# jmschrei/PyPore

Hardware: AMD Instinct MI355X
Metric: Msamples/sec segmented (SpeedyStatSplit, 10^8-sample trace); %HBM roofline (higher is better)
Workload: dtype int32/f64 (exact integer block sums of fp32 or int16 samples; decisions in fp64)

## Files before the change

pypore_amd/csrc/poreseg.hip:

```cpp
#include <hip/hip_runtime.h>

#include <algorithm>
#include <chrono>
#include <complex>
#include <cmath>
#include <cstdarg>
#include <cstdio>
#include <cstdlib>
#include <cstring>
#include <condition_variable>
#include <mutex>
#include <string>
#include <thread>
#include <tuple>
#include <vector>

#include "poreseg.h"
#include "seg_device.hpp"
#include "seg_align.hpp"
#include "seg_pairwise.hpp"
#include "seg_hmm.hpp"

using namespace ps;

// ... 62 lines not shown
    int tree_mw = 0;
    int upload_by_kernel = 1;
    int filter_fused = 1;
    int k0_waves = 0;
    float noise_k = 0.1f;
    int k0_admit = 0;
    int k0_sets = 2;
    bool chain_held = false;
    unsigned long long chain_ticket = 0;
    bool defer_sync = false;
    int scan_lds_pad = 0;
    int k0_unaligned = 1;
    int single_pass = 1;
    int gather_fused = 1;
    int download_by_kernel = 1;
    int debug = 0;
#ifdef PS_DIAG
    int dbg_phase = 0;
    int dbg_k0_nogrp = 0;
#endif
    int k0_shared = 0;
    hipEvent_t ev_front[2] = {};
    bool stream_idle = true;
    int tree_par = 1;
    int groups = 1;
    int scan_bs = 1;
    int wide_bs = 1;
    int bridge_single = 1 << 30;
    int tree_tail_pct = 0;
    int slots_pct = 100;
// ... 29 lines not shown
    DevBuf bridges, bmeta, tile_i32, sp_off, spine_items, asm_hdr, ev_first_tile;
    DevBuf bridge_ext, ext_slot, ext_list;
    DevBuf lat_state, lat_seam, lat_res;
    unsigned lat_tag_next = 1;
    unsigned lat_tag_base = 0;
    int lat_help = 1;
    int bridge_budget = BR_MAX;
    int bridge_ext_on = 1;
    HostBuf h_hdr;
    DevBuf spine_jobs, spine_scratch, spine_dense, spine_meta, tree_jobs, tree_scratch, tree_spill,
        tree_counts, items, item_pos, first_item, ev_off, bounds_off, small;
    HostBuf h_meta, h_dense, h_small, h_up;
    hipEvent_t ev[10] = {};
    int timing = 1;
    double ms[8] = {0, 0, 0, 0, 0, 0, 0, 0};
    int64_t counters[14] = {0, 0, 0, 0, 0, 0, 0, 0, 0, 0, 0, 0, 0, 0};
};

namespace {

int fail(ps_ctx *ctx, int code, const char *fmt, ...)
{
    if (ctx) {
        char buf[512];
        va_list ap;
        va_start(ap, fmt);
        vsnprintf(buf, sizeof buf, fmt, ap);
        va_end(ap);
        ctx->err = buf;
    }
    return code;
// ... 51 lines not shown
        if (c.gen[w % K0Chain::RING] == w + 1) HIP_TRY(ctx, hipStreamWaitEvent(st, c.ev[w % K0Chain::RING], 0));
    }
    return PS_OK;
}
int chain_publish(ps_ctx *ctx, int device, hipStream_t st, unsigned long long ticket)
{
    K0Chain &c = g_chain[device & 15];
    std::lock_guard<std::mutex> lk(c.mu);
    HIP_TRY(ctx, hipEventRecord(c.ev[ticket % K0Chain::RING], st));
    c.gen[ticket % K0Chain::RING] = ticket + 1;
    return PS_OK;
}
constexpr size_t SMALL_TAIL = 64 * 1024;
struct SmallLayout { unsigned long long status, work0, work1, work2, dense, stamp[12], life[9], qctl, qhead, tree_tail; AsmHeader hdr;
                     unsigned long long lat_ctl[6]; int lat_prog[LAT_D];
                     unsigned long long nt_cur; };

int make_cfg(ps_ctx *ctx, const void *d_samples, const ps_sample_format *fmt, int mw, int maxw, int W,
             double min_gain, DevCfg *c)
{
    if (!fmt) return fail(ctx, PS_ERR_ARG, "sample format is NULL");
    if (fmt->dtype != PS_DTYPE_F32 && fmt->dtype != PS_DTYPE_I16)
        return fail(ctx, PS_ERR_ARG, "unknown dtype %d", fmt->dtype);
    if (!(fmt->quantum > 0) || !std::isfinite(fmt->quantum))
        return fail(ctx, PS_ERR_ARG, "quantum must be positive and finite");
    c->samples = d_samples;
    c->dtype = fmt->dtype;
    c->off_counts = fmt->dtype == PS_DTYPE_F32 ? 0 : fmt->offset_counts;
    c->dc_counts = fmt->dtype == PS_DTYPE_F32 ? static_cast<double>(fmt->offset_counts) : 0.0;
    c->noise_k = ctx->noise_k;
    c->inv_q = static_cast<float>(1.0 / fmt->quantum);
// ... 231 lines not shown
                  : cfg.bsum != nullptr && cfg.bs_wide && ctx->tree_mw
                      ? (f32 ? launch_tree_mw<PS_DTYPE_F32 | DT_WIDE>(ctx, cfg, g, sm, n_tj, d_hdr) : launch_tree_mw<PS_DTYPE_I16 | DT_WIDE>(ctx, cfg, g, sm, n_tj, d_hdr))
                  : cfg.bsum != nullptr && cfg.bs_wide
                      ? (f32 ? launch_tree<64, PS_DTYPE_F32 | DT_WIDE>(ctx, cfg, g, sm, n_tj, d_hdr) : launch_tree<64, PS_DTYPE_I16 | DT_WIDE>(ctx, cfg, g, sm, n_tj, d_hdr))
                  : cfg.bsum != nullptr && ctx->tree_mw
                      ? (f32 ? launch_tree_mw<PS_DTYPE_F32>(ctx, cfg, g, sm, n_tj, d_hdr) : launch_tree_mw<PS_DTYPE_I16>(ctx, cfg, g, sm, n_tj, d_hdr))
                  : cfg.bsum != nullptr
                      ? (f32 ? launch_tree<64, PS_DTYPE_F32>(ctx, cfg, g, sm, n_tj, d_hdr) : launch_tree<64, PS_DTYPE_I16>(ctx, cfg, g, sm, n_tj, d_hdr))
                  : ctx->tree_nt == 512
                      ? (f32 ? launch_tree<512, PS_DTYPE_F32>(ctx, cfg, g, sm, n_tj, d_hdr) : launch_tree<512, PS_DTYPE_I16>(ctx, cfg, g, sm, n_tj, d_hdr))
                      : (f32 ? launch_tree<256, PS_DTYPE_F32>(ctx, cfg, g, sm, n_tj, d_hdr) : launch_tree<256, PS_DTYPE_I16>(ctx, cfg, g, sm, n_tj, d_hdr));
        if (lrc) return lrc;
    }
    if (ctx->timing >= 2) HIP_TRY(ctx, hipEventRecord(ctx->ev[3], ctx->stream));
    const bool fused = d_hdr != nullptr && ctx->gather_fused;
    if (fused) {
        const int64_t blocks = (n_items >> GS_LOG) + 1;
        const unsigned gg = static_cast<unsigned>(std::max<int64_t>(1, std::min<int64_t>(blocks, 1024)));
        hipLaunchKernelGGL(gather_scan_kernel, dim3(gg), dim3(1 << GS_LOG), 0, ctx->stream, ctx->items.as<Item>(),
                           ctx->tree_jobs.as<TreeJob>(), ctx->tree_counts.as<int32_t>(), ctx->tree_scratch.as<int32_t>(),
                           static_cast<long long>(n_items), d_bounds, cap, ctx->d_is_spine, d_hdr, ctx->first_item.as<int64_t>(),
                           n_ev, ctx->bounds_off.as<int64_t>());
        HIP_TRY(ctx, hipGetLastError());
    } else {
    hipLaunchKernelGGL(item_scan_kernel, dim3(1), dim3(1024), 0, ctx->stream, ctx->items.as<Item>(),
                       ctx->tree_counts.as<int32_t>(), n_items, ctx->item_pos.as<int64_t>(), d_hdr,
                       ctx->first_item.as<int64_t>(), n_ev, ctx->bounds_off.as<int64_t>());
    HIP_TRY(ctx, hipGetLastError());
    }
    if (n_items && !fused) {
        const unsigned gg = static_cast<unsigned>(d_hdr ? std::min<int64_t>(n_items, 16384) : n_items);
        hipLaunchKernelGGL(gather_kernel, dim3(gg), dim3(64), 0, ctx->stream,
                           ctx->items.as<Item>(), ctx->tree_jobs.as<TreeJob>(), ctx->tree_counts.as<int32_t>(),
                           ctx->tree_scratch.as<int32_t>(), ctx->item_pos.as<int64_t>(), n_items, d_bounds, cap, ctx->d_is_spine,
                           d_hdr);
        HIP_TRY(ctx, hipGetLastError());
    }
    const bool stats_from_digest = d_stats != nullptr && cfg.bsum != nullptr && cfg.blk_mm != nullptr;
    if (stats_from_digest) {
        const int64_t scap = cap + n_ev;
        const unsigned sg = static_cast<unsigned>(std::min<int64_t>(std::max<int64_t>(scap, 1), 8192));
        if (cfg.dtype == PS_DTYPE_F32)
            hipLaunchKernelGGL(segstat_bs_kernel<PS_DTYPE_F32>, dim3(sg), dim3(64), 0, ctx->stream, cfg, ctx->ev_off.as<int64_t>(),
                               ctx->ev_len.as<int64_t>(), n_ev, d_bounds, ctx->bounds_off.as<int64_t>(), d_stats, scap,
                               reinterpret_cast<unsigned *>(&sm->status), d_hdr);
        else
            hipLaunchKernelGGL(segstat_bs_kernel<PS_DTYPE_I16>, dim3(sg), dim3(64), 0, ctx->stream, cfg, ctx->ev_off.as<int64_t>(),
                               ctx->ev_len.as<int64_t>(), n_ev, d_bounds, ctx->bounds_off.as<int64_t>(), d_stats, scap,
                               reinterpret_cast<unsigned *>(&sm->status), d_hdr);
        HIP_TRY(ctx, hipGetLastError());
        if (ctx->timing >= 2) HIP_TRY(ctx, hipEventRecord(ctx->ev[4], ctx->stream));
    }
    const bool one_copy = ctx->bounds_off.p == ctx->small.as<char>() + sizeof(SmallLayout);
    if (one_copy) {
        HIP_TRY(ctx, ctx->h_small.reserve(sizeof(SmallLayout) + evb));
        void *h_dev = nullptr;
        if (ctx->download_by_kernel && hipHostGetDevicePointer(&h_dev, ctx->h_small.p, 0) != hipSuccess) { h_dev = nullptr; (void)hipGetLastError(); }
        if (h_dev) {
            static_assert(sizeof(SmallLayout) % 8 == 0, "the status block is copied in 8-byte words");
            const long long nw = static_cast<long long>((sizeof(SmallLayout) + evb) / 8);
            hipLaunchKernelGGL(download_kernel, dim3(static_cast<unsigned>(std::min<long long>((nw + 255) / 256, 64))), dim3(256), 0, ctx->stream,
                               ctx->small.as<unsigned long long>(), static_cast<unsigned long long *>(h_dev), nw);
            HIP_TRY(ctx, hipGetLastError());
        } else {
            HIP_TRY(ctx, hipMemcpyAsync(ctx->h_small.p, ctx->small.p, sizeof(SmallLayout) + evb, hipMemcpyDeviceToHost, ctx->stream));
        }
    } else {
        HIP_TRY(ctx, ctx->h_meta.reserve(evb));
        HIP_TRY(ctx, hipMemcpyAsync(ctx->h_meta.p, ctx->bounds_off.p, evb, hipMemcpyDeviceToHost, ctx->stream));
        HIP_TRY(ctx, hipMemcpyAsync(ctx->h_small.p, ctx->small.p, sizeof(SmallLayout), hipMemcpyDeviceToHost, ctx->stream));
    }
    if (ctx->timing >= 1) HIP_TRY(ctx, hipEventRecord(ctx->ev[9], ctx->stream));
    HIP_TRY(ctx, hipStreamSynchronize(ctx->stream));
    {
        float seq = 0;
// ... 37 lines not shown
        }
    }
    ctx->counters[0] = static_cast<int64_t>(hs.work0);
    ctx->counters[1] = static_cast<int64_t>(hs.work1);
    ctx->counters[5] = static_cast<int64_t>(hs.work2 & 0xffffffffULL) + static_cast<int64_t>(hs.work2 >> 32);
    ctx->counters[6] = static_cast<int64_t>(hs.work2 >> 32);
#ifndef PS_STAMP
    for (int k = 0; k < 3; ++k) ctx->counters[8 + k] = static_cast<int64_t>(hs.life[3 * k + 1]);
    ctx->counters[11] = cfg.bsum ? static_cast<int64_t>(hs.stamp[0]) : -1;
    ctx->nt_seen = cfg.bsum && cfg.nt_log ? static_cast<int64_t>(hs.nt_cur) : -1;
#else
    ctx->nt_seen = -1;
#endif
    ctx->counters[12] = static_cast<int64_t>(hs.lat_ctl[4]);
    ctx->counters[13] = static_cast<int64_t>(hs.lat_ctl[5]);
#ifdef PS_STAMP
    {
        static const char *nm[12] = {"level", "sweep", "drain", "decide", "contend", "setup", "exact", "outside", "-", "-", "-", "-"};
        unsigned long long tot = 0;
        for (int i = 0; i < 8; ++i) tot += hs.stamp[i];
        fprintf(stderr, "[poreseg stamps] lane-0 cycles summed over waves (spine+bridge+tree):");
        for (int i = 0; i < 8; ++i) fprintf(stderr, " %s=%.1f%%", nm[i], 100.0 * hs.stamp[i] / (tot ? tot : 1));
        fprintf(stderr, " total=%llu cycles, windows=%llu -> %.0f cycles/window\n", tot, hs.work0, (double)tot / (hs.work0 ? hs.work0 : 1));
        fprintf(stderr, "[poreseg stamps] rows swept %llu, non-empty drains %llu, blocks drained %llu, hit-like windows %llu\n",
                hs.stamp[8], hs.stamp[9], hs.stamp[10], hs.stamp[11]);
        fprintf(stderr, "[poreseg stamps] blocks queued although not prunable (first block of a window, variance floor): %llu\n", hs.stamp[6]);
        for (int k = 0; k < 3; ++k)
            fprintf(stderr, "[poreseg stamps] %s: longest workgroup %llu cycles, windows %llu, sum of lifetimes %llu cycles\n",
                    k == 0 ? "spine" : k == 1 ? "bridge" : "tree", hs.life[3 * k], hs.life[3 * k + 1], hs.life[3 * k + 2]);
    }
// ... 31 lines not shown

LatHelp lat_help_of(ps_ctx *ctx, const DevCfg &cfg, SmallLayout *sm)
{
    if (!ctx->lat_help || cfg.bsum == nullptr || !ctx->lat_res.p) return LAT_NONE;
    LatHelp h;
    h.ctl = sm->lat_ctl;
    h.state = ctx->lat_state.as<unsigned long long>();
    h.seam = ctx->lat_seam.as<int>();
    h.prog = sm->lat_prog;
    h.res = ctx->lat_res.as<unsigned long long>();
    h.tag_base = ctx->lat_tag_base;
    h.stay = ctx->lat_help == 2 ? 1 : 0;
    return h;
}

template <int DT> int launch_bridge_la(ps_ctx *ctx, const DevCfg &cfg, unsigned nj, SmallLayout *sm)
{
    const unsigned grid = std::min(nj, resident_slots(ctx, bridge_la_kernel<DT>, 64 * BR_LA, 0));
    hipLaunchKernelGGL((bridge_la_kernel<DT>), dim3(grid), dim3(64 * BR_LA), 0, ctx->stream, cfg,
                       ctx->spine_jobs.as<SpineJob>(), ctx->spine_scratch.as<int2>(), ctx->spine_meta.as<int4>(),
                       ctx->bridges.as<int2>(), ctx->bmeta.as<int4>(), reinterpret_cast<unsigned *>(&sm->status),
                       &sm->work0, static_cast<int>(nj), nullptr, nullptr, nullptr, 0, ctx->bridge_budget, static_cast<int>(EXT_MAX),
                       lat_help_of(ctx, cfg, sm));
    HIP_TRY(ctx, hipGetLastError());
    return PS_OK;
}

template <int NT, int DT> int launch_bridge(ps_ctx *ctx, const DevCfg &cfg, unsigned nj, SmallLayout *sm)
{
    const size_t lds = NT == 64 ? static_cast<size_t>(ctx->scan_lds_pad) : lds_bytes_for(cfg.lds_cap, NT);
    HIP_TRY(ctx, set_dyn_lds(ctx, reinterpret_cast<const void *>(bridge_kernel<NT, DT>), static_cast<int>(lds)));
    const unsigned grid = std::min(nj, resident_slots(ctx, bridge_kernel<NT, DT>, NT, lds));
    hipLaunchKernelGGL((bridge_kernel<NT, DT>), dim3(grid), dim3(NT), lds, ctx->stream, cfg,
                       ctx->spine_jobs.as<SpineJob>(), ctx->spine_scratch.as<int2>(), ctx->spine_meta.as<int4>(),
                       ctx->bridges.as<int2>(), ctx->bmeta.as<int4>(), reinterpret_cast<unsigned *>(&sm->status),
                       &sm->work0, static_cast<int>(nj), ctx->bridge_single, ctx->bridge_budget,
                       NT == 64 ? lat_help_of(ctx, cfg, sm) : LAT_NONE);
    HIP_TRY(ctx, hipGetLastError());
    return PS_OK;
}

int device_stitch_batch_(ps_ctx *ctx, const DevCfg &cfg_in, int bs_mode, const int64_t *ev_start, const int64_t *ev_len, int32_t n_ev, int mw, int W,
                        int32_t *d_bounds, int64_t cap, int64_t *h_bounds_off, ps_segstat *d_stats,
                        std::chrono::steady_clock::time_point t_begin, bool digest_ready = false)
{
    DevCfg cfg = cfg_in;
    const bool use_bs = bs_mode != 0;
    const bool wide = bs_mode == 2;
    cfg.bs_wide = wide ? 1 : 0;
    int64_t L = ctx->tile_len;
    ps_ctx::TileCache &tc = ctx->tile_cache;
    const size_t evb = (static_cast<size_t>(n_ev) + 1) * sizeof(int64_t);
// ... 49 lines not shown
        HIP_TRY(ctx, ctx->up_dev.reserve(up_bytes + 64));
        char *up = ctx->h_up.as<char>();
        if (nj) std::memcpy(up, jobs.data(), nj * sizeof(SpineJob));
        std::memcpy(up + jb, ev_first_tile.data(), evb);
        std::memcpy(up + jb + evb, ev_start, evb - sizeof(int64_t));
        std::memcpy(up + jb + 2 * evb, ev_len, evb - sizeof(int64_t));
        std::memcpy(up + jb + 3 * evb, boff.data(), evb);
        tc.n_ev = n_ev; tc.mw = mw; tc.W = W; tc.L = L; tc.use_bs = use_bs;
        tc.ev_start.assign(ev_start, ev_start + n_ev); tc.ev_len.assign(ev_len, ev_len + n_ev);
        tc.nj = nj; tc.jb = jb; tc.up_bytes = up_bytes; tc.list_entries = list_entries; tc.total_len = total_len;
        tc.sample_end = sample_end; tc.nb_total = boff[n_ev];
    }
    const size_t nj = tc.nj, jb = tc.jb, up_bytes = tc.up_bytes;
    const int64_t list_entries = tc.list_entries, total_len = tc.total_len, sample_end = tc.sample_end;
    ctx->counters[2] = static_cast<int64_t>(nj);
    const int64_t max_items = list_entries + static_cast<int64_t>(nj) * BR_MAX;
    const int64_t tscratch_bound = total_len / mw + max_items + 1;

    HIP_TRY(ctx, ctx->spine_scratch.reserve(std::max<int64_t>(1, list_entries) * sizeof(int2)));
    HIP_TRY(ctx, ctx->spine_meta.reserve(std::max<size_t>(4, nj) * sizeof(int4)));
    HIP_TRY(ctx, ctx->bridges.reserve(std::max<size_t>(1, nj) * BR_MAX * sizeof(int2)));
    if (use_bs && ctx->lat_help) {
        const size_t res_bytes = static_cast<size_t>(LAT_D) * LAT_C * sizeof(unsigned long long);
        HIP_TRY(ctx, ctx->lat_state.reserve(LAT_D * sizeof(unsigned long long)));
        HIP_TRY(ctx, ctx->lat_seam.reserve(LAT_D * sizeof(int)));
        HIP_TRY(ctx, ctx->lat_res.reserve_zeroed(res_bytes, ctx->stream));
        if (ctx->lat_tag_next + 2u * LAT_TAGS >= (1u << 24)) {
            HIP_TRY(ctx, hipMemsetAsync(ctx->lat_res.p, 0, res_bytes, ctx->stream));
            ctx->stream_idle = false;
            ctx->lat_tag_next = 1;
// ... 160 lines not shown
                  : ctx->spine_nt == 512
                      ? (f32 ? launch_spine<512, PS_DTYPE_F32>(ctx, cfg, g, sm, true) : launch_spine<512, PS_DTYPE_I16>(ctx, cfg, g, sm, true))
                      : (f32 ? launch_spine<1024, PS_DTYPE_F32>(ctx, cfg, g, sm, true) : launch_spine<1024, PS_DTYPE_I16>(ctx, cfg, g, sm, true));
        if (lrc) return lrc;
        if (ctx->timing >= 2) HIP_TRY(ctx, hipEventRecord(ctx->ev[6], ctx->stream));
        lrc = ctx->spine_nt == 256
                  ? (f32 ? launch_bridge<256, PS_DTYPE_F32>(ctx, cfg, g, sm) : launch_bridge<256, PS_DTYPE_I16>(ctx, cfg, g, sm))
                  : (f32 ? launch_bridge<512, PS_DTYPE_F32>(ctx, cfg, g, sm) : launch_bridge<512, PS_DTYPE_I16>(ctx, cfg, g, sm));
        if (lrc) return lrc;
    }
    if (ctx->timing >= 2) HIP_TRY(ctx, hipEventRecord(ctx->ev[1], ctx->stream));
    int *ti = ctx->tile_i32.as<int>();
    const size_t njp = std::max<size_t>(1, nj);
    const size_t tile_lds = (nj + 1) * sizeof(long long) + 4 * nj * sizeof(int);
    const int use_lds = tile_lds <= 150 * 1024;
    if (use_lds)
        HIP_TRY(ctx, set_dyn_lds(ctx, reinterpret_cast<const void *>(assemble_tiles_kernel), static_cast<int>(tile_lds)));
    AsmHeader hd = {};
    int rc = PS_OK;
    int64_t items_cap = max_items;
    int slots_used = 0, ext_stride = EXT_MAX;
    for (int round = 0;; ++round) {
        hipLaunchKernelGGL(assemble_tiles_kernel, dim3(1), dim3(1024), use_lds ? tile_lds : 0, ctx->stream,
                           static_cast<int>(nj), ctx->spine_meta.as<int4>(), ctx->bmeta.as<int4>(),
                           ctx->ev_first_tile.as<int64_t>(), n_ev, ti, ti + njp, ti + 2 * njp, ti + 3 * njp,
                           ctx->sp_off.as<long long>(), ctx->first_item.as<int64_t>(), ctx->asm_hdr.as<AsmHeader>(),
                           static_cast<long long>(items_cap), use_lds, reinterpret_cast<const unsigned *>(&sm->status));
        HIP_TRY(ctx, hipGetLastError());
        const AsmHeader *d_hdr = ctx->asm_hdr.as<AsmHeader>();
        if (items_cap > 0) {
            const unsigned ag = static_cast<unsigned>(std::min<int64_t>((items_cap + 255) / 256, 2048));
            hipLaunchKernelGGL(assemble_items_kernel, dim3(ag), dim3(256), 0,
                               ctx->stream, ctx->spine_jobs.as<SpineJob>(), static_cast<int>(nj), ctx->spine_meta.as<int4>(),
                               ctx->spine_scratch.as<int2>(), ctx->bridges.as<int2>(), ti + 3 * njp,
                               ctx->sp_off.as<long long>(), static_cast<long long>(items_cap), mw, W, ctx->tree_jobs.as<TreeJob>(),
                               ctx->items.as<Item>(), ctx->tree_counts.as<int32_t>(), d_hdr, cfg.bsum != nullptr ? cfg.ev_info : nullptr,
                               ctx->bridge_ext.as<int2>(), ctx->ext_slot.as<int>(), ext_stride);
            HIP_TRY(ctx, hipGetLastError());
        }
        if (ctx->timing >= 2 && round == 0) HIP_TRY(ctx, hipEventRecord(ctx->ev[5], ctx->stream));
        rc = finish_batch(ctx, cfg, static_cast<size_t>(items_cap), items_cap, n_ev, d_bounds, cap, h_bounds_off, d_stats, t_begin,
                          d_hdr, &hd, use_bs);
        if (rc != RC_FALLBACK || !use_bs || !nj || round == EXT_ROUNDS || !ctx->bridge_ext_on) break;
        HIP_TRY(ctx, ctx->h_meta.reserve(2 * nj * sizeof(int4)));
        int4 *h_bm = ctx->h_meta.as<int4>(), *h_mt = h_bm + nj;
// ... 250 lines not shown
    else if (n == "prune") ctx->prune = value != 0;
    else if (n == "scan_bs") ctx->scan_bs = value != 0;
    else if (n == "near_tie_log" && value >= 0 && value <= (int64_t(1) << 30)) ctx->nt_cap = value;
    else if (n == "groups") ctx->groups = value != 0;
    else if (n == "tree_par") ctx->tree_par = value != 0;
    else if (n == "k0_waves" && value >= 0 && value <= 16) ctx->k0_waves = static_cast<int>(value);
    else if (n == "k0_shared") ctx->k0_shared = value != 0;
    else if (n == "k0_admit" && value >= 0) ctx->k0_admit = static_cast<int>(value);
    else if (n == "bridge_ext" && (value == 0 || value == 1)) ctx->bridge_ext_on = static_cast<int>(value);
    else if (n == "lat_help" && value >= 0 && value <= 2) ctx->lat_help = static_cast<int>(value);
    else if (n == "shared_device" && value >= 0 && value <= 4096) {
        const bool sh = value > 1;
        ctx->k0_waves = sh ? 1 : 0;
        ctx->lat_help = sh ? 0 : 1;
        ctx->k0_admit = value > 3 ? 3 : 0;
    }
    else if (n == "hmm_bp_budget" && value >= 1) ctx->hmm_bp_budget = value;
    else if (n == "hmm_fb_budget" && value >= 1) ctx->hmm_fb_budget = value;
    else if (n == "pairwise_budget" && value >= 1) ctx->pw_budget = value;
    else if (n == "hmm_expect_lds") ctx->hmm_expect_lds = value != 0;
    else if (n == "single_pass") ctx->single_pass = value != 0;
    else if (n == "gather_fused") ctx->gather_fused = value != 0;
    else if (n == "download_by_kernel") ctx->download_by_kernel = value != 0;
    else if (n == "debug") ctx->debug = value != 0;
    else if (n == "k0_unaligned") ctx->k0_unaligned = value != 0 ? k0_unaligned_probe(ctx->device, ctx->stream) : 0;
    else if (n == "slots_pct" && value >= 1 && value <= 100) ctx->slots_pct = static_cast<int>(value);
    else if (n == "tree_jobs_per_wave" && value >= 0 && value <= 1024) ctx->tree_jobs_per_wave = static_cast<int>(value);
    else if (n == "noise_k_ppm" && value >= 0) ctx->noise_k = static_cast<float>(static_cast<double>(value) * 1.0e-6);
#ifdef PS_DIAG
    else if (n == "dbg_phase" && value >= 0 && value <= 2) ctx->dbg_phase = static_cast<int>(value);
    else if (n == "dbg_k0_nogrp") ctx->dbg_k0_nogrp = value != 0;
    else if (n == "cu_mask" && ctx->own_stream)
        return diag_mask_stream(ctx, &ctx->stream, static_cast<int>(value & 0xfff), static_cast<int>((value >> 12) & 0xfff),
                                static_cast<int>((value >> 24) & 0xff), ((value >> 32) & 1) != 0);
    else if (n == "k0_sets" && value >= 2 && value <= 4) ctx->k0_sets = static_cast<int>(value);
    else if (n == "scan_lds_pad" && value >= 0 && value <= 65536) ctx->scan_lds_pad = static_cast<int>(value);
    else if (n == "rep_eval" && value >= 1) ctx->rep_eval = static_cast<int>(value);
    else if (n == "rep_stage" && value >= 1) ctx->rep_stage = static_cast<int>(value);
// ... 761 lines not shown
    }
    auto key = [](const ps_near_tie &a) { return std::make_tuple(a.event, a.window_start, a.window_end, a.split); };
    std::sort(sites.begin(), sites.end(), [&](const ps_near_tie &a, const ps_near_tie &b) { return key(a) < key(b); });
    sites.erase(std::unique(sites.begin(), sites.end(), [&](const ps_near_tie &a, const ps_near_tie &b) { return key(a) == key(b); }),
                sites.end());
    *n_out = static_cast<int64_t>(sites.size());
    if (sites.size() > static_cast<size_t>(cap)) return PS_ERR_CAPACITY;
    std::copy(sites.begin(), sites.end(), out);
    return PS_OK;
}

int ps_get_timings(const ps_ctx *ctx, double *ms, int32_t n_ms, int64_t *counters, int32_t n_counters)
{
    if (!ctx) return PS_ERR_ARG;
    for (int i = 0; i < n_ms && ms; ++i) ms[i] = i < 8 ? ctx->ms[i] : 0.0;
    for (int i = 0; i < n_counters && counters; ++i) counters[i] = i < 14 ? ctx->counters[i] : 0;
    return PS_OK;
}

const int64_t *ps_counters(const ps_ctx *ctx) { return ctx ? ctx->counters : nullptr; }

int ps_synth_trace(ps_ctx *ctx, void *d_out, int32_t dtype, int64_t n, uint64_t seed,
                   const int64_t *h_seg_end, const int32_t *h_level_counts, int64_t nseg)
{
    if (!ctx) return PS_ERR_ARG;
    if (!d_out || n < 0 || nseg < 1 || !h_seg_end || !h_level_counts) return fail(ctx, PS_ERR_ARG, "bad argument");
    if (h_seg_end[nseg - 1] < n) return fail(ctx, PS_ERR_ARG, "segment table does not cover n");
    HIP_TRY(ctx, hipSetDevice(ctx->device));
    const size_t b1 = static_cast<size_t>(nseg) * sizeof(int64_t), b2 = static_cast<size_t>(nseg) * sizeof(int32_t);
    HIP_TRY(ctx, ctx->tree_scratch.reserve(b1 + b2));
    char *d = ctx->tree_scratch.as<char>();
// ... 808 lines not shown
```

pypore_amd/csrc/seg_device.hpp:

```cpp
#pragma once
#include <hip/hip_runtime.h>
#include <stdint.h>
#include "poreseg.h"

namespace ps {

constexpr int LDS_STACK = 128;
constexpr int MAX_WAVES = 16;
constexpr int OBUF = 256;
constexpr int BR_MAX = 256;
constexpr int LST_MAX = 256;
constexpr int LAT_D = 256;
constexpr int LAT_W = 16;
constexpr int LAT_C = 2048;
constexpr int LAT_TAGS = 4096;
struct LatHelp {
    unsigned long long *ctl;
    unsigned long long *state;
    int *seam;
    int *prog;
    unsigned long long *res;
    unsigned tag_base;
    int stay;
};
// ... 1175 lines not shown

enum : int { BR_NONE = 0, BR_JOINED = 1, BR_ENDED = 2, BR_FAIL = 3, BR_DEFER = 4,
              BR_FAIL_REACHED = 5 };
__device__ __forceinline__ int2 bridge_at(const int2 *bridges, const int2 *ext, const int *ext_slot, int ext_stride, int g, int i)
{
    return i < BR_MAX ? bridges[static_cast<long long>(g) * BR_MAX + i]
                      : ext[static_cast<long long>(ext_slot[g]) * ext_stride + (i - BR_MAX)];
}
constexpr int BR_PATIENCE = 3;

template <int NT, int DT>
__global__ __launch_bounds__(NT, (NT == 64 ? PS_BRIDGE_MINW : 4)) PS_BRIDGE_REGS void bridge_kernel(DevCfg c, const SpineJob *jobs, const int2 *lists,
                                                       const int4 *meta, int2 *bridges, int4 *bmeta,
                                                       unsigned *status, unsigned long long *work, int n_jobs, int max_single,
                                                       int budget = BR_MAX,
                                                       LatHelp lat = LAT_NONE)
{
    extern __shared__ int ys[];
    __shared__ SharedT<NT> sh;
    if (c.bsum != nullptr && (*status & ST_WIDE_RANGE) != 0u) return;
    unsigned bad = 0;
    Work wk = PS_WORK_INIT;
    for (int g = blockIdx.x; g < n_jobs; g += gridDim.x) {
        const SpineJob job = jobs[g];
        const int4 m = meta[g];
        const bool last_tile = (g - job.first_tile) == job.ntiles - 1;
        if (last_tile || m.y != 0) {
            if (threadIdx.x == 0) bmeta[g] = make_int4(0, -1, 0, BR_NONE);
            continue;
        }
        if (m.x == 0 && g != job.first_tile) {
// ... 19 lines not shown
            if (a == uj.start) found = -1;
            else {
                int lo = 0, hi = ccnt - 1;
                while (lo <= hi) {
                    const int mid = (lo + hi) >> 1;
                    const int v = mid < SharedT<NT>::LN ? sh.lst[mid] : lists[uj.out_off + mid].x;
                    if (v == a) { found = mid; break; }
                    if (v < a) lo = mid + 1; else hi = mid - 1;
                }
            }
            if (found != -2 && u != g) { st = BR_JOINED; jt = u; ji = found; break; }
            if (step == budget) break;
            if (NT == 64 && c.bsum != nullptr && cnt >= max_single) { st = BR_DEFER; jt = 0; break; }
            int kind;
            const int s = find_split<NT, DT, false>(c, ys, job.base, a, job.end, step == 0 ? m.z : 0, kind, sh, bad, wk, job.end, er,
                                                    0x7fffffffffffffffLL, (NT == 64 && c.bsum != nullptr) ? BR_PATIENCE : 0x7fffffff);
            if (kind == KIND_NONE) { st = BR_ENDED; break; }
            if (kind == KIND_STOP) { st = BR_DEFER; jt = s; break; }
            if (threadIdx.x == 0) sh.obuf[cnt] = make_int2(s, kind);
            ++cnt;
            a = s;
        }
        __syncthreads();
        for (int i = threadIdx.x; i < cnt; i += NT) bridges[static_cast<int64_t>(g) * BR_MAX + i] = sh.obuf[i];
        if (threadIdx.x == 0) {
            bmeta[g] = make_int4(cnt, jt, ji, st);
            if (st == BR_DEFER && lat.ctl != nullptr && c.half > 0) {
                const long long ps0 = static_cast<long long>(a) + static_cast<long long>(jt + LAT_W) * c.half;
                if (ps0 < static_cast<long long>(job.end) - 2LL * c.mw) {
                    int u = static_cast<int>(ps0 / job.tile_len);
                    if (u > job.ntiles - 1) u = job.ntiles - 1;
                    const int4 mu = meta[job.first_tile + u];
                    if (mu.x == 0 && mu.y == 0) atomicAdd(&lat.ctl[0], 1ull);
                }
            }
        }
        __syncthreads();
    }
    flush(bad, wk, status, work, 1);
}

// ... 598 lines not shown
        if (item.job >= 0) {
            cnt = counts[item.job];
            const int32_t *src = scratch + jobs[item.job].out_off;
            for (int i = threadIdx.x; i < cnt; i += 64)
                if (p + i < cap) { bounds[p + i] = src[i]; if (is_spine) is_spine[p + i] = 0; }
        }
        if (threadIdx.x == 0 && p + cnt < cap) { bounds[p + cnt] = item.anchor; if (is_spine) is_spine[p + cnt] = 1; }
    }
}



__global__ __launch_bounds__(256) void gather_scan_kernel(const Item *items, const TreeJob *jobs, const int32_t *counts,
                                                          const int32_t *scratch, long long n_items_host, int32_t *bounds,
                                                          int64_t cap, uint8_t *is_spine, const AsmHeader *hdr,
                                                          const int64_t *first_item, int32_t n_ev, int64_t *bounds_off)
{
    constexpr int GS = 1 << GS_LOG;
    __shared__ long long wsum[GS / 64];
    __shared__ int ws[GS / 64];
    __shared__ long long pos_s[GS];
    __shared__ int ev_lo_s, ev_hi_s;
    const bool failed = hdr && hdr->fail;
    const long long n_items = dev_count(hdr, n_items_host);
    const int32_t *blk = counts + n_items_host;
    const int tid = threadIdx.x, lane = tid & 63, wave = tid >> 6;
    if (failed) {
        for (long long e = blockIdx.x * static_cast<long long>(GS) + tid; e <= n_ev; e += gridDim.x * static_cast<long long>(GS)) bounds_off[e] = 0;
        return;
    }
    const long long nb = (n_items >> GS_LOG) + 1;
    for (long long b = blockIdx.x; b < nb; b += gridDim.x) {
        long long part = 0;
        for (long long k = tid; k < b; k += GS) part += blk[k];
#pragma unroll
        for (int d = 32; d >= 1; d >>= 1) part += __shfl_down(part, d);
        const long long i = (b << GS_LOG) + tid;
        const bool have = i < n_items;
        Item it = {-1, 0};
        int cnt = 0;
        if (have) { it = items[i]; if (it.job >= 0) cnt = counts[it.job]; }
        const int v = have ? cnt + 1 : 0;
        int inc = v;
#pragma unroll
        for (int d = 1; d < 64; d <<= 1) { const int u = __shfl_up(inc, d); if (lane >= d) inc += u; }
        if (lane == 0) wsum[wave] = part;
// ... 16 lines not shown
        unsigned long long big = __ballot(cnt > 16);
        while (big) {
            const int l = __builtin_ctzll(big);
            big &= big - 1ull;
            const long long pl = __shfl(p, l);
            const int cl = __shfl(cnt, l);
            const int32_t *sl = reinterpret_cast<const int32_t *>(__shfl(reinterpret_cast<unsigned long long>(src), l));
            for (int k = lane; k < cl; k += 64)
                if (pl + k < cap) { bounds[pl + k] = sl[k]; if (is_spine) is_spine[pl + k] = 0; }
        }
        if (cnt <= 16)
            for (int k = 0; k < cnt; ++k)
                if (p + k < cap) { bounds[p + k] = src[k]; if (is_spine) is_spine[p + k] = 0; }
        if (have && p + cnt < cap) { bounds[p + cnt] = it.anchor; if (is_spine) is_spine[p + cnt] = 1; }
    }
}

__global__ __launch_bounds__(256) void download_kernel(const unsigned long long *src, unsigned long long *dst_host, long long n_words)
{
    for (long long i = blockIdx.x * 256LL + threadIdx.x; i < n_words; i += gridDim.x * 256LL) dst_host[i] = src[i];
}

__device__ __forceinline__ void chunk_exscan2(long long v1, long long v2, long long &e1, long long &e2,
                                              long long *wsum , long long *carry )
{
    const int lane = threadIdx.x & 63, wave = threadIdx.x >> 6;
    long long i1 = v1, i2 = v2;
#pragma unroll
    for (int d = 1; d < 64; d <<= 1) {
        const long long u1 = __shfl_up(i1, d), u2 = __shfl_up(i2, d);
        if (lane >= d) { i1 += u1; i2 += u2; }
    }
    if (lane == 63) { wsum[wave] = i1; wsum[16 + wave] = i2; }
    __syncthreads();
    long long b1 = carry[0], b2 = carry[1];
    for (int w = 0; w < wave; ++w) { b1 += wsum[w]; b2 += wsum[16 + w]; }
    e1 = b1 + i1 - v1; e2 = b2 + i2 - v2;
    __syncthreads();
    if (threadIdx.x == 1023) { carry[0] = b1 + i1; carry[1] = b2 + i2; }
    __syncthreads();
}

__global__ __launch_bounds__(1024) void assemble_tiles_kernel(
    int n_tiles, const int4 *meta, int4 *bmeta, const int64_t *ev_first_tile, int n_ev,
    int *g_reach, int *g_jump_a, int *g_jump_b, int *entry_out, long long *sp_off_out,
    int64_t *first_item, AsmHeader *hdr, long long max_items, int use_lds, const unsigned *status)
{
    if ((*status & ST_WIDE_RANGE) != 0u) {
        if (threadIdx.x == 0) { hdr->n_items = 0; hdr->n_jobs = 0; hdr->tscratch = 0; hdr->fail = 1; hdr->pad = 0; }
        return;
    }
    extern __shared__ long long dyn_lds[];
    __shared__ long long wsum[32];
    __shared__ long long carry[2];
    __shared__ int fail_s;
    const int tid = threadIdx.x;
    long long *sp_off = use_lds ? dyn_lds : sp_off_out;
    int *lds_i = reinterpret_cast<int *>(dyn_lds + (n_tiles + 1));
    int *reach = use_lds ? lds_i : g_reach;
    int *ja = use_lds ? lds_i + n_tiles : g_jump_a;
    int *jb = use_lds ? lds_i + 2 * n_tiles : g_jump_b;
    int *entry = use_lds ? lds_i + 3 * n_tiles : entry_out;
    if (tid == 0) { fail_s = 0; carry[0] = 0; carry[1] = 0; }
    for (int g = tid; g < n_tiles; g += 1024) {
// ... 36 lines not shown
            if (c < 0) fail_s = 1;
        }
        long long e1, e2;
        chunk_exscan2(n, 0, e1, e2, wsum, carry);
        if (g < n_tiles) sp_off[g] = e1;
    }
    const long long n_items = carry[0];
    if (tid == 0) sp_off[n_tiles] = n_items;
    __syncthreads();
    for (int e = tid; e <= n_ev; e += 1024) first_item[e] = sp_off[ev_first_tile[e]];
    if (use_lds)
        for (int g = tid; g <= n_tiles; g += 1024) {
            sp_off_out[g] = sp_off[g];
            if (g < n_tiles) entry_out[g] = entry[g];
        }
    if (tid == 0) {
        hdr->n_items = n_items;
        hdr->n_jobs = n_items;
        hdr->tscratch = 0;
        hdr->fail = (fail_s || n_items > max_items) ? 1 : 0;
    }
}

__global__ __launch_bounds__(256) void assemble_items_kernel(
    const SpineJob *jobs, int n_tiles, const int4 *meta, const int2 *lists, const int2 *bridges,
    const int *entry, const long long *sp_off, long long n_items_host, int mw, int W,
    TreeJob *tjobs, Item *items, int32_t *counts, const AsmHeader *hdr, const int4 *ev_info,
    const int2 *ext = nullptr, const int *ext_slot = nullptr, int ext_stride = EXT_MAX)
{
    const long long n_items = dev_count(hdr, n_items_host);
    for (long long b = blockIdx.x * 256LL + threadIdx.x; b <= (n_items >> GS_LOG); b += gridDim.x * 256LL) counts[n_items_host + b] = 0;
    for (long long i = blockIdx.x * 256LL + threadIdx.x; i < n_items; i += gridDim.x * 256LL) {
    int lo = 0, hi = n_tiles - 1;
    while (lo < hi) {
        const int mid = (lo + hi) >> 1;
        if (sp_off[mid + 1] > i) hi = mid; else lo = mid + 1;
    }
    const int g = lo;
    const int k = static_cast<int>(i - sp_off[g]);
    const int en = entry[g], cnt = meta[g].x;
    const SpineJob jb2 = jobs[g];
    int2 el;
    int pred;
    if (k < cnt - en) {
        el = lists[jb2.out_off + en + k];
        pred = (en + k) > 0 ? lists[jb2.out_off + en + k - 1].x : jb2.start;
    } else {
        const int kb = k - (cnt - en);
        el = bridge_at(bridges, ext, ext_slot, ext_stride, g, kb);
        pred = kb > 0 ? bridge_at(bridges, ext, ext_slot, ext_stride, g, kb - 1).x : (cnt > 0 ? lists[jb2.out_off + cnt - 1].x : jb2.start);
    }
    const bool has = el.y == KIND_HIT || el.y == KIND_LATE;
    Item it;
    it.anchor = el.x;
    it.job = has ? static_cast<int32_t>(i) : -1;
    items[i] = it;
    TreeJob tj;
    tj.base = jb2.base;
    tj.start = pred;
    tj.end = el.x;
    tj.j0 = left_child_j0(pred, el.x, W, W / 2);
    tj.out_cap = has ? (el.x - pred) / mw + 1 : 0;
    tj.out_off = (jb2.vbase + pred) / mw + i;
    tj.pad_ = 0;
    if (ev_info) {
        const int4 info = ev_info[jb2.ev];
        tj.m = info.x;
        tj.pad_ = info.y;
        tj.boff = (static_cast<long long>(static_cast<unsigned>(info.w)) << 32) | static_cast<unsigned>(info.z);
    } else { tj.m = 0; tj.boff = 0; }
    tjobs[i] = tj;
    counts[i] = 0;
    }
}


constexpr int DET_NT = 256;
constexpr int DET_PER = 16;
constexpr int DET_CHUNK = DET_NT * DET_PER;

template <int DT>
__device__ __forceinline__ bool below_thr(const DevCfg &c, int k, double thr)
{
    return static_cast<double>(k) * c.q < thr;
}

template <int DT>
__global__ __launch_bounds__(DET_NT) void edge_scan_kernel(DevCfg c, int64_t n, double thr, int *tics,
// ... 298 lines not shown
```

Before: 513,700.

## Fuse item assembly into tile stitch, fold download into gather, inline bridges

Adds an assemble_fused_kernel that runs item assembly inside the single-block tile-stitch kernel using the LDS prefix offsets, with four items unrolled per thread, so the separate assemble_items launch disappears. The last gather_scan block, found through an atomic ticket, now copies the status block to pinned host memory, which removes the separate download kernel. When the context is shared, the bridge lookahead launch is skipped and the bridge kernel gets unlimited patience; a defer counter is added as well. The trade-off is that item assembly now runs on one 1024-thread block instead of a grid, which may be slower when there are many items, in exchange for fewer kernel launches.

```diff
diff --git a/pypore_amd/csrc/poreseg.hip b/pypore_amd/csrc/poreseg.hip
--- a/pypore_amd/csrc/poreseg.hip
+++ b/pypore_amd/csrc/poreseg.hip
@@ -100,6 +100,10 @@
     int single_pass = 1;
     int gather_fused = 1;
     int download_by_kernel = 1;
+    int bridge_inline = 1;
+    int stitch_fused = 1;
+    int gather_download = 1;
+    int shared_n = 0;
     int debug = 0;
 #ifdef PS_DIAG
     int dbg_phase = 0;
@@ -159,7 +163,7 @@
     hipEvent_t ev[10] = {};
     int timing = 1;
     double ms[8] = {0, 0, 0, 0, 0, 0, 0, 0};
-    int64_t counters[14] = {0, 0, 0, 0, 0, 0, 0, 0, 0, 0, 0, 0, 0, 0};
+    int64_t counters[16] = {0, 0, 0, 0, 0, 0, 0, 0, 0, 0, 0, 0, 0, 0, 0, 0};
 };
 
 namespace {
@@ -241,7 +245,8 @@
 constexpr size_t SMALL_TAIL = 64 * 1024;
 struct SmallLayout { unsigned long long status, work0, work1, work2, dense, stamp[12], life[9], qctl, qhead, tree_tail; AsmHeader hdr;
                      unsigned long long lat_ctl[6]; int lat_prog[LAT_D];
-                     unsigned long long nt_cur; };
+                     unsigned long long nt_cur;
+                     unsigned long long n_defer, gs_ticket; };
 
 int make_cfg(ps_ctx *ctx, const void *d_samples, const ps_sample_format *fmt, int mw, int maxw, int W,
              double min_gain, DevCfg *c)
@@ -503,13 +508,24 @@
     }
     if (ctx->timing >= 2) HIP_TRY(ctx, hipEventRecord(ctx->ev[3], ctx->stream));
     const bool fused = d_hdr != nullptr && ctx->gather_fused;
+    const bool stats_from_digest = d_stats != nullptr && cfg.bsum != nullptr && cfg.blk_mm != nullptr;
+    const bool one_copy = ctx->bounds_off.p == ctx->small.as<char>() + sizeof(SmallLayout);
+    void *h_dev = nullptr;
+    if (one_copy) {
+        HIP_TRY(ctx, ctx->h_small.reserve(sizeof(SmallLayout) + evb));
+        if (ctx->download_by_kernel && hipHostGetDevicePointer(&h_dev, ctx->h_small.p, 0) != hipSuccess) { h_dev = nullptr; (void)hipGetLastError(); }
+    }
+    static_assert(sizeof(SmallLayout) % 8 == 0, "the status block is copied in 8-byte words");
+    const long long dl_words = static_cast<long long>((sizeof(SmallLayout) + evb) / 8);
+    const bool gather_dl = fused && ctx->gather_download && h_dev != nullptr && !stats_from_digest;
     if (fused) {
         const int64_t blocks = (n_items >> GS_LOG) + 1;
         const unsigned gg = static_cast<unsigned>(std::max<int64_t>(1, std::min<int64_t>(blocks, 1024)));
         hipLaunchKernelGGL(gather_scan_kernel, dim3(gg), dim3(1 << GS_LOG), 0, ctx->stream, ctx->items.as<Item>(),
                            ctx->tree_jobs.as<TreeJob>(), ctx->tree_counts.as<int32_t>(), ctx->tree_scratch.as<int32_t>(),
                            static_cast<long long>(n_items), d_bounds, cap, ctx->d_is_spine, d_hdr, ctx->first_item.as<int64_t>(),
-                           n_ev, ctx->bounds_off.as<int64_t>());
+                           n_ev, ctx->bounds_off.as<int64_t>(), gather_dl ? &sm->gs_ticket : nullptr,
+                           ctx->small.as<unsigned long long>(), static_cast<unsigned long long *>(h_dev), dl_words);
         HIP_TRY(ctx, hipGetLastError());
     } else {
     hipLaunchKernelGGL(item_scan_kernel, dim3(1), dim3(1024), 0, ctx->stream, ctx->items.as<Item>(),
@@ -525,7 +541,6 @@
                            d_hdr);
         HIP_TRY(ctx, hipGetLastError());
     }
-    const bool stats_from_digest = d_stats != nullptr && cfg.bsum != nullptr && cfg.blk_mm != nullptr;
     if (stats_from_digest) {
         const int64_t scap = cap + n_ev;
         const unsigned sg = static_cast<unsigned>(std::min<int64_t>(std::max<int64_t>(scap, 1), 8192));
@@ -540,14 +555,10 @@
         HIP_TRY(ctx, hipGetLastError());
         if (ctx->timing >= 2) HIP_TRY(ctx, hipEventRecord(ctx->ev[4], ctx->stream));
     }
-    const bool one_copy = ctx->bounds_off.p == ctx->small.as<char>() + sizeof(SmallLayout);
-    if (one_copy) {
-        HIP_TRY(ctx, ctx->h_small.reserve(sizeof(SmallLayout) + evb));
-        void *h_dev = nullptr;
-        if (ctx->download_by_kernel && hipHostGetDevicePointer(&h_dev, ctx->h_small.p, 0) != hipSuccess) { h_dev = nullptr; (void)hipGetLastError(); }
+    if (gather_dl) {
+    } else if (one_copy) {
         if (h_dev) {
-            static_assert(sizeof(SmallLayout) % 8 == 0, "the status block is copied in 8-byte words");
-            const long long nw = static_cast<long long>((sizeof(SmallLayout) + evb) / 8);
+            const long long nw = dl_words;
             hipLaunchKernelGGL(download_kernel, dim3(static_cast<unsigned>(std::min<long long>((nw + 255) / 256, 64))), dim3(256), 0, ctx->stream,
                                ctx->small.as<unsigned long long>(), static_cast<unsigned long long *>(h_dev), nw);
             HIP_TRY(ctx, hipGetLastError());
@@ -615,6 +626,7 @@
 #endif
     ctx->counters[12] = static_cast<int64_t>(hs.lat_ctl[4]);
     ctx->counters[13] = static_cast<int64_t>(hs.lat_ctl[5]);
+    ctx->counters[14] = static_cast<int64_t>(hs.n_defer);
 #ifdef PS_STAMP
     {
         static const char *nm[12] = {"level", "sweep", "drain", "decide", "contend", "setup", "exact", "outside", "-", "-", "-", "-"};
@@ -676,8 +688,12 @@
     return h;
 }
 
+bool bridge_inline_of(const ps_ctx *ctx) { return ctx->bridge_inline && ctx->shared_n > 1 && ctx->bridge_single >= (1 << 30); }
+
 template <int DT> int launch_bridge_la(ps_ctx *ctx, const DevCfg &cfg, unsigned nj, SmallLayout *sm)
 {
+    if (bridge_inline_of(ctx)) return PS_OK;
+    ctx->counters[15] += 1;
     const unsigned grid = std::min(nj, resident_slots(ctx, bridge_la_kernel<DT>, 64 * BR_LA, 0));
     hipLaunchKernelGGL((bridge_la_kernel<DT>), dim3(grid), dim3(64 * BR_LA), 0, ctx->stream, cfg,
                        ctx->spine_jobs.as<SpineJob>(), ctx->spine_scratch.as<int2>(), ctx->spine_meta.as<int4>(),
@@ -697,7 +713,7 @@
                        ctx->spine_jobs.as<SpineJob>(), ctx->spine_scratch.as<int2>(), ctx->spine_meta.as<int4>(),
                        ctx->bridges.as<int2>(), ctx->bmeta.as<int4>(), reinterpret_cast<unsigned *>(&sm->status),
                        &sm->work0, static_cast<int>(nj), ctx->bridge_single, ctx->bridge_budget,
-                       NT == 64 ? lat_help_of(ctx, cfg, sm) : LAT_NONE);
+                       NT == 64 ? lat_help_of(ctx, cfg, sm) : LAT_NONE, bridge_inline_of(ctx) ? 0x7fffffff : BR_PATIENCE, &sm->n_defer);
     HIP_TRY(ctx, hipGetLastError());
     return PS_OK;
 }
@@ -777,6 +793,8 @@
     const size_t nj = tc.nj, jb = tc.jb, up_bytes = tc.up_bytes;
     const int64_t list_entries = tc.list_entries, total_len = tc.total_len, sample_end = tc.sample_end;
     ctx->counters[2] = static_cast<int64_t>(nj);
+    ctx->counters[14] = 0;
+    ctx->counters[15] = 0;
     const int64_t max_items = list_entries + static_cast<int64_t>(nj) * BR_MAX;
     const int64_t tscratch_bound = total_len / mw + max_items + 1;
 
@@ -967,13 +985,27 @@
     const size_t njp = std::max<size_t>(1, nj);
     const size_t tile_lds = (nj + 1) * sizeof(long long) + 4 * nj * sizeof(int);
     const int use_lds = tile_lds <= 150 * 1024;
+    const bool stitch_fused = ctx->stitch_fused && use_lds;
     if (use_lds)
-        HIP_TRY(ctx, set_dyn_lds(ctx, reinterpret_cast<const void *>(assemble_tiles_kernel), static_cast<int>(tile_lds)));
+        HIP_TRY(ctx, set_dyn_lds(ctx, stitch_fused ? reinterpret_cast<const void *>(assemble_fused_kernel) : reinterpret_cast<const void *>(assemble_tiles_kernel),
+                                 static_cast<int>(tile_lds)));
     AsmHeader hd = {};
     int rc = PS_OK;
     int64_t items_cap = max_items;
     int slots_used = 0, ext_stride = EXT_MAX;
     for (int round = 0;; ++round) {
+        const bool fuse_now = stitch_fused && items_cap > 0;
+        if (fuse_now) {
+            const AsmItemsArgs ia = {ctx->spine_jobs.as<SpineJob>(), ctx->spine_meta.as<int4>(), ctx->spine_scratch.as<int2>(), ctx->bridges.as<int2>(),
+                                     static_cast<long long>(items_cap), mw, W, ctx->tree_jobs.as<TreeJob>(), ctx->items.as<Item>(),
+                                     ctx->tree_counts.as<int32_t>(), cfg.bsum != nullptr ? cfg.ev_info : nullptr,
+                                     ctx->bridge_ext.as<int2>(), ctx->ext_slot.as<int>(), ext_stride};
+            hipLaunchKernelGGL(assemble_fused_kernel, dim3(1), dim3(1024), tile_lds, ctx->stream,
+                               static_cast<int>(nj), ctx->spine_meta.as<int4>(), ctx->bmeta.as<int4>(),
+                               ctx->ev_first_tile.as<int64_t>(), n_ev, ti, ti + njp, ti + 2 * njp, ti + 3 * njp,
+                               ctx->sp_off.as<long long>(), ctx->first_item.as<int64_t>(), ctx->asm_hdr.as<AsmHeader>(),
+                               static_cast<long long>(items_cap), use_lds, reinterpret_cast<const unsigned *>(&sm->status), ia);
+        } else
         hipLaunchKernelGGL(assemble_tiles_kernel, dim3(1), dim3(1024), use_lds ? tile_lds : 0, ctx->stream,
                            static_cast<int>(nj), ctx->spine_meta.as<int4>(), ctx->bmeta.as<int4>(),
                            ctx->ev_first_tile.as<int64_t>(), n_ev, ti, ti + njp, ti + 2 * njp, ti + 3 * njp,
@@ -981,7 +1013,7 @@
                            static_cast<long long>(items_cap), use_lds, reinterpret_cast<const unsigned *>(&sm->status));
         HIP_TRY(ctx, hipGetLastError());
         const AsmHeader *d_hdr = ctx->asm_hdr.as<AsmHeader>();
-        if (items_cap > 0) {
+        if (items_cap > 0 && !fuse_now) {
             const unsigned ag = static_cast<unsigned>(std::min<int64_t>((items_cap + 255) / 256, 2048));
             hipLaunchKernelGGL(assemble_items_kernel, dim3(ag), dim3(256), 0,
                                ctx->stream, ctx->spine_jobs.as<SpineJob>(), static_cast<int>(nj), ctx->spine_meta.as<int4>(),
@@ -1262,6 +1294,7 @@
         ctx->k0_waves = sh ? 1 : 0;
         ctx->lat_help = sh ? 0 : 1;
         ctx->k0_admit = value > 3 ? 3 : 0;
+        ctx->shared_n = static_cast<int>(value);
     }
     else if (n == "hmm_bp_budget" && value >= 1) ctx->hmm_bp_budget = value;
     else if (n == "hmm_fb_budget" && value >= 1) ctx->hmm_fb_budget = value;
@@ -1270,6 +1303,9 @@
     else if (n == "single_pass") ctx->single_pass = value != 0;
     else if (n == "gather_fused") ctx->gather_fused = value != 0;
     else if (n == "download_by_kernel") ctx->download_by_kernel = value != 0;
+    else if (n == "bridge_inline") ctx->bridge_inline = value != 0;
+    else if (n == "stitch_fused") ctx->stitch_fused = value != 0;
+    else if (n == "gather_download") ctx->gather_download = value != 0;
     else if (n == "debug") ctx->debug = value != 0;
     else if (n == "k0_unaligned") ctx->k0_unaligned = value != 0 ? k0_unaligned_probe(ctx->device, ctx->stream) : 0;
     else if (n == "slots_pct" && value >= 1 && value <= 100) ctx->slots_pct = static_cast<int>(value);
@@ -2061,7 +2097,7 @@
 {
     if (!ctx) return PS_ERR_ARG;
     for (int i = 0; i < n_ms && ms; ++i) ms[i] = i < 8 ? ctx->ms[i] : 0.0;
-    for (int i = 0; i < n_counters && counters; ++i) counters[i] = i < 14 ? ctx->counters[i] : 0;
+    for (int i = 0; i < n_counters && counters; ++i) counters[i] = i < 16 ? ctx->counters[i] : 0;
     return PS_OK;
 }
 
diff --git a/pypore_amd/csrc/seg_device.hpp b/pypore_amd/csrc/seg_device.hpp
--- a/pypore_amd/csrc/seg_device.hpp
+++ b/pypore_amd/csrc/seg_device.hpp
@@ -1213,7 +1213,9 @@
                                                        const int4 *meta, int2 *bridges, int4 *bmeta,
                                                        unsigned *status, unsigned long long *work, int n_jobs, int max_single,
                                                        int budget = BR_MAX,
-                                                       LatHelp lat = LAT_NONE)
+                                                       LatHelp lat = LAT_NONE,
+                                                       int patience = BR_PATIENCE,
+                                                       unsigned long long *n_defer = nullptr)
 {
     extern __shared__ int ys[];
     __shared__ SharedT<NT> sh;
@@ -1263,7 +1265,7 @@
             if (NT == 64 && c.bsum != nullptr && cnt >= max_single) { st = BR_DEFER; jt = 0; break; }
             int kind;
             const int s = find_split<NT, DT, false>(c, ys, job.base, a, job.end, step == 0 ? m.z : 0, kind, sh, bad, wk, job.end, er,
-                                                    0x7fffffffffffffffLL, (NT == 64 && c.bsum != nullptr) ? BR_PATIENCE : 0x7fffffff);
+                                                    0x7fffffffffffffffLL, (NT == 64 && c.bsum != nullptr) ? patience : 0x7fffffff);
             if (kind == KIND_NONE) { st = BR_ENDED; break; }
             if (kind == KIND_STOP) { st = BR_DEFER; jt = s; break; }
             if (threadIdx.x == 0) sh.obuf[cnt] = make_int2(s, kind);
@@ -1274,6 +1276,7 @@
         for (int i = threadIdx.x; i < cnt; i += NT) bridges[static_cast<int64_t>(g) * BR_MAX + i] = sh.obuf[i];
         if (threadIdx.x == 0) {
             bmeta[g] = make_int4(cnt, jt, ji, st);
+            if (st == BR_DEFER && n_defer != nullptr) atomicAdd(n_defer, 1ull);
             if (st == BR_DEFER && lat.ctl != nullptr && c.half > 0) {
                 const long long ps0 = static_cast<long long>(a) + static_cast<long long>(jt + LAT_W) * c.half;
                 if (ps0 < static_cast<long long>(job.end) - 2LL * c.mw) {
@@ -1902,9 +1905,12 @@
 __global__ __launch_bounds__(256) void gather_scan_kernel(const Item *items, const TreeJob *jobs, const int32_t *counts,
                                                           const int32_t *scratch, long long n_items_host, int32_t *bounds,
                                                           int64_t cap, uint8_t *is_spine, const AsmHeader *hdr,
-                                                          const int64_t *first_item, int32_t n_ev, int64_t *bounds_off)
+                                                          const int64_t *first_item, int32_t n_ev, int64_t *bounds_off,
+                                                          unsigned long long *ticket = nullptr, const unsigned long long *dl_src = nullptr,
+                                                          unsigned long long *dl_dst_host = nullptr, long long dl_words = 0)
 {
     constexpr int GS = 1 << GS_LOG;
+    __shared__ int last_s;
     __shared__ long long wsum[GS / 64];
     __shared__ int ws[GS / 64];
     __shared__ long long pos_s[GS];
@@ -1913,11 +1919,9 @@
     const long long n_items = dev_count(hdr, n_items_host);
     const int32_t *blk = counts + n_items_host;
     const int tid = threadIdx.x, lane = tid & 63, wave = tid >> 6;
-    if (failed) {
+    if (failed)
         for (long long e = blockIdx.x * static_cast<long long>(GS) + tid; e <= n_ev; e += gridDim.x * static_cast<long long>(GS)) bounds_off[e] = 0;
-        return;
-    }
-    const long long nb = (n_items >> GS_LOG) + 1;
+    const long long nb = failed ? 0 : (n_items >> GS_LOG) + 1;
     for (long long b = blockIdx.x; b < nb; b += gridDim.x) {
         long long part = 0;
         for (long long k = tid; k < b; k += GS) part += blk[k];
@@ -1964,6 +1968,17 @@
                 if (p + k < cap) { bounds[p + k] = src[k]; if (is_spine) is_spine[p + k] = 0; }
         if (have && p + cnt < cap) { bounds[p + cnt] = it.anchor; if (is_spine) is_spine[p + cnt] = 1; }
     }
+    if (ticket != nullptr) {
+        __threadfence();
+        __syncthreads();
+        if (tid == 0) last_s = __hip_atomic_fetch_add(ticket, 1ull, __ATOMIC_RELAXED, __HIP_MEMORY_SCOPE_AGENT) == gridDim.x - 1ull;
+        __syncthreads();
+        if (last_s) {
+            __threadfence();
+            if (tid == 0) lat_st(ticket, 0ull);
+            for (long long i = tid; i < dl_words; i += GS) dl_dst_host[i] = lat_ld(dl_src + i);
+        }
+    }
 }
 
 __global__ __launch_bounds__(256) void download_kernel(const unsigned long long *src, unsigned long long *dst_host, long long n_words)
@@ -1991,13 +2006,25 @@
     __syncthreads();
 }
 
-__global__ __launch_bounds__(1024) void assemble_tiles_kernel(
+struct AsmItemsArgs {
+    const SpineJob *jobs; const int4 *meta; const int2 *lists; const int2 *bridges;
+    long long n_items_host; int mw, W;
+    TreeJob *tjobs; Item *items; int32_t *counts; const int4 *ev_info;
+    const int2 *ext; const int *ext_slot; int ext_stride;
+};
+template <int U>
+__device__ __forceinline__ void assemble_items_run(const AsmItemsArgs &p, int n_tiles, long long n_items, long long first, long long stride,
+                                                   const int *entry, const long long *sp_off);
+
+template <bool ITEMS>
+__device__ __forceinline__ void assemble_tiles_run(
     int n_tiles, const int4 *meta, int4 *bmeta, const int64_t *ev_first_tile, int n_ev,
     int *g_reach, int *g_jump_a, int *g_jump_b, int *entry_out, long long *sp_off_out,
-    int64_t *first_item, AsmHeader *hdr, long long max_items, int use_lds, const unsigned *status)
+    int64_t *first_item, AsmHeader *hdr, long long max_items, int use_lds, const unsigned *status, const AsmItemsArgs &it)
 {
     if ((*status & ST_WIDE_RANGE) != 0u) {
         if (threadIdx.x == 0) { hdr->n_items = 0; hdr->n_jobs = 0; hdr->tscratch = 0; hdr->fail = 1; hdr->pad = 0; }
+        if (ITEMS && threadIdx.x == 0) it.counts[it.n_items_host] = 0;
         return;
     }
     extern __shared__ long long dyn_lds[];
@@ -2064,11 +2091,90 @@
             sp_off_out[g] = sp_off[g];
             if (g < n_tiles) entry_out[g] = entry[g];
         }
+    const bool failed = fail_s || n_items > max_items;
     if (tid == 0) {
         hdr->n_items = n_items;
         hdr->n_jobs = n_items;
         hdr->tscratch = 0;
-        hdr->fail = (fail_s || n_items > max_items) ? 1 : 0;
+        hdr->fail = failed ? 1 : 0;
+    }
+    if constexpr (ITEMS) {
+        __syncthreads();
+        assemble_items_run<4>(it, n_tiles, failed ? 0 : n_items, tid, 1024, entry, sp_off);
+    }
+}
+
+__global__ __launch_bounds__(1024) void assemble_tiles_kernel(
+    int n_tiles, const int4 *meta, int4 *bmeta, const int64_t *ev_first_tile, int n_ev,
+    int *g_reach, int *g_jump_a, int *g_jump_b, int *entry_out, long long *sp_off_out,
+    int64_t *first_item, AsmHeader *hdr, long long max_items, int use_lds, const unsigned *status)
+{
+    assemble_tiles_run<false>(n_tiles, meta, bmeta, ev_first_tile, n_ev, g_reach, g_jump_a, g_jump_b, entry_out, sp_off_out, first_item, hdr,
+                              max_items, use_lds, status, AsmItemsArgs{});
+}
+
+template <int U>
+__device__ __forceinline__ void assemble_items_run(const AsmItemsArgs &p, int n_tiles, long long n_items, long long first, long long stride,
+                                                   const int *entry, const long long *sp_off)
+{
+    for (long long b = first; b <= (n_items >> GS_LOG); b += stride) p.counts[p.n_items_host + b] = 0;
+    for (long long i0 = first; i0 < n_items; i0 += stride * U) {
+        long long ii[U];
+        int g[U], k[U], en[U], cnt[U], pred[U];
+        SpineJob jb2[U];
+        int2 el[U];
+        int4 info[U];
+#pragma unroll
+        for (int u = 0; u < U; ++u) {
+            ii[u] = i0 + u * stride < n_items ? i0 + u * stride : n_items - 1;
+            int lo = 0, hi = n_tiles - 1;
+            while (lo < hi) {
+                const int mid = (lo + hi) >> 1;
+                if (sp_off[mid + 1] > ii[u]) hi = mid; else lo = mid + 1;
+            }
+            g[u] = lo;
+            k[u] = static_cast<int>(ii[u] - sp_off[lo]);
+        }
+#pragma unroll
+        for (int u = 0; u < U; ++u) { en[u] = entry[g[u]]; cnt[u] = p.meta[g[u]].x; jb2[u] = p.jobs[g[u]]; }
+#pragma unroll
+        for (int u = 0; u < U; ++u) {
+            if (k[u] < cnt[u] - en[u]) {
+                el[u] = p.lists[jb2[u].out_off + en[u] + k[u]];
+                pred[u] = (en[u] + k[u]) > 0 ? p.lists[jb2[u].out_off + en[u] + k[u] - 1].x : jb2[u].start;
+            } else {
+                const int kb = k[u] - (cnt[u] - en[u]);
+                el[u] = bridge_at(p.bridges, p.ext, p.ext_slot, p.ext_stride, g[u], kb);
+                pred[u] = kb > 0 ? bridge_at(p.bridges, p.ext, p.ext_slot, p.ext_stride, g[u], kb - 1).x
+                                 : (cnt[u] > 0 ? p.lists[jb2[u].out_off + cnt[u] - 1].x : jb2[u].start);
+            }
+            info[u] = p.ev_info ? p.ev_info[jb2[u].ev] : make_int4(0, 0, 0, 0);
+        }
+#pragma unroll
+        for (int u = 0; u < U; ++u) {
+            const long long i = i0 + u * stride;
+            if (i >= n_items) break;
+            const bool has = el[u].y == KIND_HIT || el[u].y == KIND_LATE;
+            Item it;
+            it.anchor = el[u].x;
+            it.job = has ? static_cast<int32_t>(i) : -1;
+            p.items[i] = it;
+            TreeJob tj;
+            tj.base = jb2[u].base;
+            tj.start = pred[u];
+            tj.end = el[u].x;
+            tj.j0 = left_child_j0(pred[u], el[u].x, p.W, p.W / 2);
+            tj.out_cap = has ? (el[u].x - pred[u]) / p.mw + 1 : 0;
+            tj.out_off = (jb2[u].vbase + pred[u]) / p.mw + i;
+            tj.pad_ = 0;
+            if (p.ev_info) {
+                tj.m = info[u].x;
+                tj.pad_ = info[u].y;
+                tj.boff = (static_cast<long long>(static_cast<unsigned>(info[u].w)) << 32) | static_cast<unsigned>(info[u].z);
+            } else { tj.m = 0; tj.boff = 0; }
+            p.tjobs[i] = tj;
+            p.counts[i] = 0;
+        }
     }
 }
 
@@ -2078,50 +2184,17 @@
     TreeJob *tjobs, Item *items, int32_t *counts, const AsmHeader *hdr, const int4 *ev_info,
     const int2 *ext = nullptr, const int *ext_slot = nullptr, int ext_stride = EXT_MAX)
 {
-    const long long n_items = dev_count(hdr, n_items_host);
-    for (long long b = blockIdx.x * 256LL + threadIdx.x; b <= (n_items >> GS_LOG); b += gridDim.x * 256LL) counts[n_items_host + b] = 0;
-    for (long long i = blockIdx.x * 256LL + threadIdx.x; i < n_items; i += gridDim.x * 256LL) {
-    int lo = 0, hi = n_tiles - 1;
-    while (lo < hi) {
-        const int mid = (lo + hi) >> 1;
-        if (sp_off[mid + 1] > i) hi = mid; else lo = mid + 1;
-    }
-    const int g = lo;
-    const int k = static_cast<int>(i - sp_off[g]);
-    const int en = entry[g], cnt = meta[g].x;
-    const SpineJob jb2 = jobs[g];
-    int2 el;
-    int pred;
-    if (k < cnt - en) {
-        el = lists[jb2.out_off + en + k];
-        pred = (en + k) > 0 ? lists[jb2.out_off + en + k - 1].x : jb2.start;
-    } else {
-        const int kb = k - (cnt - en);
-        el = bridge_at(bridges, ext, ext_slot, ext_stride, g, kb);
-        pred = kb > 0 ? bridge_at(bridges, ext, ext_slot, ext_stride, g, kb - 1).x : (cnt > 0 ? lists[jb2.out_off + cnt - 1].x : jb2.start);
-    }
-    const bool has = el.y == KIND_HIT || el.y == KIND_LATE;
-    Item it;
-    it.anchor = el.x;
-    it.job = has ? static_cast<int32_t>(i) : -1;
-    items[i] = it;
-    TreeJob tj;
-    tj.base = jb2.base;
-    tj.start = pred;
-    tj.end = el.x;
-    tj.j0 = left_child_j0(pred, el.x, W, W / 2);
-    tj.out_cap = has ? (el.x - pred) / mw + 1 : 0;
-    tj.out_off = (jb2.vbase + pred) / mw + i;
-    tj.pad_ = 0;
-    if (ev_info) {
-        const int4 info = ev_info[jb2.ev];
-        tj.m = info.x;
-        tj.pad_ = info.y;
-        tj.boff = (static_cast<long long>(static_cast<unsigned>(info.w)) << 32) | static_cast<unsigned>(info.z);
-    } else { tj.m = 0; tj.boff = 0; }
-    tjobs[i] = tj;
-    counts[i] = 0;
-    }
+    const AsmItemsArgs p = {jobs, meta, lists, bridges, n_items_host, mw, W, tjobs, items, counts, ev_info, ext, ext_slot, ext_stride};
+    assemble_items_run<1>(p, n_tiles, dev_count(hdr, n_items_host), blockIdx.x * 256LL + threadIdx.x, gridDim.x * 256LL, entry, sp_off);
+}
+
+__global__ __launch_bounds__(1024) void assemble_fused_kernel(
+    int n_tiles, const int4 *meta, int4 *bmeta, const int64_t *ev_first_tile, int n_ev,
+    int *g_reach, int *g_jump_a, int *g_jump_b, int *entry_out, long long *sp_off_out,
+    int64_t *first_item, AsmHeader *hdr, long long max_items, int use_lds, const unsigned *status, AsmItemsArgs it)
+{
+    assemble_tiles_run<true>(n_tiles, meta, bmeta, ev_first_tile, n_ev, g_reach, g_jump_a, g_jump_b, entry_out, sp_off_out, first_item, hdr,
+                             max_items, use_lds, status, it);
 }
 
 
```

After: 318,200. 38.1% lower.
